# soedinglab/spacedust

Hardware: AMD Instinct MI355X
Metric: clustersearch throughput (genome-pairs/s; SW GCUPS alongside) (higher is better)
Workload: dtype int16

## Files before the change

spacedust_amd/csrc/hip/sd_sw.hip:

```cpp
#include "sd_common.h"
#include <unistd.h>


#include <algorithm>
#include <cmath>
#include <cstring>
#include <memory>
#include <omp.h>
#include <numeric>

#include "../host/sd_host.h"
#include "sd_sw_pk.h"

namespace {

using sdpk::SwTask;

template <int RT>
__global__ void __launch_bounds__(64)
sw_score_kernel(const SwTask *__restrict__ tasks, uint32_t nTasks, const uint8_t *__restrict__ qRes,
                const int8_t *__restrict__ qBias, const uint8_t *__restrict__ tRes, const int8_t *__restrict__ mat,
                int go, int ge, int32_t *__restrict__ out, uint2 *__restrict__ boundary,
                const uint32_t *__restrict__ order ,
                const int8_t *__restrict__ qProf ) {
// ... 601 lines not shown
    int i = qLen - 1, j = tLen - 1, state = 2;
    char *o = bt + tk.btOff + (qLen + tLen + 2);
    int len = 0, ids = 0;
    bool bad = false;
    bool going = have && reached && (i > 0 || j > 0);
    const int sh = grp * 32;
    while (__ballot(going)) {
        {
            const int ii = i - l, jj = j - l;
            bool ok = going && state == 2 && (ii > 0 || jj > 0) && ii >= 0 && jj >= 0;
            int x = ii - band;
            x = x > 0 ? x : 0;
            x = jj - x;
            ok = ok && x >= 0 && x < width_d;
            bool same = false;
            if (ok) {
                const int byte = dirs[(size_t) 16 * ii + (x >> 1)];
                const int code = (x & 1) ? (byte >> 4) : (byte & 15);
                ok = (code & 12) == 0;
                same = sq[ii] == st[jj];
            }
            const uint32_t okMask = (uint32_t) (__ballot(ok) >> sh);
            const uint32_t sameMask = (uint32_t) (__ballot(same) >> sh);
            const int run = okMask == 0xFFFFFFFFu ? 32 : __builtin_ctz(~okMask);
            const uint32_t runMask = run == 32 ? 0xFFFFFFFFu : ((1u << run) - 1u);
            if (l < run) o[-1 - l] = 'M';
            ids += __builtin_popcount(sameMask & runMask);
            i -= run;
            j -= run;
            o -= run;
            len += run;
        }
        if (going && (i > 0 || j > 0)) {
            if (i < 0 || j < 0) bad = true;
            int x = i - band;
            x = x > 0 ? x : 0;
            x = j - x;
            if (x < 0 || x >= width_d) bad = true;
            if (!bad) {
                const int byte = dirs[(size_t) 16 * i + (x >> 1)];
                const int code = (x & 1) ? (byte >> 4) : (byte & 15);
                int dcode;
                const int dE = (code & 1) ? 3 : 2, dF = (code & 2) ? 5 : 4;
                if (state == 0) dcode = dE;
                else if (state == 1) dcode = dF;
                else dcode = (code & 4) ? dE : ((code & 8) ? dF : 1);
                char c;
                switch (dcode) {
                    case 1: ids += (sq[i] == st[j]); --i; --j; state = 2; c = 'M'; break;
                    case 2: --i; state = 0; c = 'I'; break;
                    case 3: --i; state = 2; c = 'I'; break;
                    case 4: --j; state = 1; c = 'D'; break;
                    default: --j; state = 2; c = 'D'; break;
                }
                --o;
                if (l == 0) *o = c;
                len++;
            }
        }
        going = going && !bad && (i > 0 || j > 0);
    }
    if (!have || !reached || l != 0) return;
    if (bad || i != 0 || j != 0) {
        res[2 * id] = -1;
        return;
    }
    ids += (sq[0] == st[0]);
    *--o = 'M';
    len++;
    res[2 * id] = len;
    res[2 * id + 1] = ids;
}

template <int RT, int LW, bool MULTI, bool WIDE, bool SHARED>
void launchScorePk(sd_ctx *ctx, const SwTask *dTasks, const uint32_t *dOrder, uint32_t n, const sd_seqset *q,
                   const sd_seqset *t, const int8_t *dMat, int go, int ge, int32_t *dOut, uint2 *dBound) {
    if (n == 0) return;
    constexpr uint32_t perWave = 2 * (64 / LW);
    dim3 grid((n + perWave - 1) / perWave), block(64);
    hipLaunchKernelGGL((sdpk::sw_score_pk_kernel<RT, LW, MULTI, WIDE, SHARED>), grid, block, 0, ctx->stream, dTasks, n, q->dRes, q->dBias,
                       t->dRes, dMat, go, ge, dOut, dBound, dOrder, (const int8_t *) q->dProf);
}

template <int RT, bool SHARED>
void launchScorePkAligned(sd_ctx *ctx, const SwTask *dTasks, const uint32_t *dOrder, uint32_t n, const sd_seqset *q, const sd_seqset *t,
                          const int8_t *dMat, int go, int ge, int32_t *dOut) {
    if (n == 0) return;
    constexpr uint32_t perWave = 4;
    dim3 grid((n + perWave - 1) / perWave), block(64);
    hipLaunchKernelGGL((sdpk::sw_score_pk_aligned_kernel<RT, SHARED>), grid, block, 0, ctx->stream, dTasks, n, q->dRes, q->dBias, t->dRes,
                       dMat, go, ge, dOut, dOrder, (const int8_t *) q->dProf);
}

int rtClass(int n) {
    if (n <= 128) return 4;
    if (n <= 256) return 8;
    if (n <= 512) return 16;
    return 32;
}

template <int RT>
void launchScore(sd_ctx *ctx, const SwTask *dTasks, uint32_t n, const sd_seqset *q, const sd_seqset *t,
                 const int8_t *dMat, int go, int ge, int32_t *dOut, uint2 *dBound) {
    if (n == 0) return;
    dim3 grid((n + 1) / 2), block(64);
    hipLaunchKernelGGL(sw_score_kernel<RT>, grid, block, 0, ctx->stream, dTasks, n, q->dRes, q->dBias, t->dRes, dMat,
                       go, ge, dOut, dBound, (const uint32_t *) nullptr, (const int8_t *) q->dProf);
}

template <int RT>
void launchScoreIdx(sd_ctx *ctx, const SwTask *dTasks, const uint32_t *dOrder, uint32_t n, const sd_seqset *q,
                    const sd_seqset *t, const int8_t *dMat, int go, int ge, int32_t *dOut, uint2 *dBound) {
    if (n == 0) return;
    dim3 grid((n + 1) / 2), block(64);
    hipLaunchKernelGGL(sw_score_kernel<RT>, grid, block, 0, ctx->stream, dTasks, n, q->dRes, q->dBias, t->dRes, dMat,
                       go, ge, dOut, dBound, dOrder, (const int8_t *) q->dProf);
}

int runScoreTasks(sd_ctx *ctx, std::vector<SwTask> &tasks, const sd_seqset *q, const sd_seqset *t, const int8_t *dMat,
                  int go, int ge, std::vector<int32_t> &hOut, uint32_t nSlots, uint64_t *cells, const char *tag = "a") {
    hOut.assign((size_t) nSlots * 3, 0);
    if (tasks.empty()) return SD_OK;
    HostScope hsAll(ctx, "score.total");
    const size_t n = tasks.size();
    constexpr int NB = 4 * 1024;
    auto keyOf = [](const SwTask &t) {
        const int c = rtClass(t.n);
        const int ci = c == 4 ? 0 : (c == 8 ? 1 : (c == 16 ? 2 : 3));
        return (uint32_t) ci * 1024u + (uint32_t) (1023 - std::min(t.tL >> 4, 1023));
    };
    SwTask *sorted = nullptr;
    SD_HIP(ctx, pinGet(ctx, (std::string("sw.tasks.") + tag).c_str(), n, &sorted));
    uint64_t boundTotal = 0, cellSum = 0;
    size_t classBegin[5] = {0, 0, 0, 0, 0};
    {
        int T = 1;
#pragma omp parallel
        {
#pragma omp single
            T = omp_get_num_threads();
        }
        T = std::max(1, std::min(T, 64));
        std::vector<uint32_t> hist((size_t) T * NB, 0);
#pragma omp parallel num_threads(T) reduction(+ : cellSum)
        {
            const int th = omp_get_thread_num();
            const size_t lo = n * th / T, hi = n * (th + 1) / T;
            uint32_t *hh = &hist[(size_t) th * NB];
            for (size_t i = lo; i < hi; i++) {
                hh[keyOf(tasks[i])]++;
                cellSum += (uint64_t) tasks[i].n * (uint64_t) tasks[i].tL;
            }
        }
        uint64_t run = 0;
        for (int bkt = 0; bkt < NB; bkt++) {
            if ((bkt & 1023) == 0) classBegin[bkt >> 10] = run;
            for (int th = 0; th < T; th++) {
                const uint32_t c = hist[(size_t) th * NB + bkt];
                hist[(size_t) th * NB + bkt] = (uint32_t) run;
                run += c;
            }
        }
        classBegin[4] = run;
#pragma omp parallel num_threads(T)
        {
            const int th = omp_get_thread_num();
            const size_t lo = n * th / T, hi = n * (th + 1) / T;
            uint32_t *hh = &hist[(size_t) th * NB];
            for (size_t i = lo; i < hi; i++) sorted[hh[keyOf(tasks[i])]++] = tasks[i];
        }
    }
    *cells += cellSum;
    for (size_t i = classBegin[3]; i < classBegin[4]; i++) {
        if (sorted[i].n > 1024) {
            sorted[i].boundOff = boundTotal;
            boundTotal += (uint64_t) sorted[i].tL;
        }
    }
    SwTask *dTasks = nullptr;
    int32_t *dOut = nullptr;
    uint2 *dBound = nullptr;
    int32_t *hPin = nullptr;
    SD_HIP(ctx, wsGet(ctx, "sw.tasks", n, &dTasks));
    SD_HIP(ctx, wsGet(ctx, "sw.out", (size_t) nSlots * 3, &dOut));
    SD_HIP(ctx, wsGet(ctx, "sw.bound", std::max<uint64_t>(boundTotal, 1), &dBound));
    SD_HIP(ctx, pinGet(ctx, "sw.hout", (size_t) nSlots * 3, &hPin));
    SD_HIP(ctx, hipMemcpyAsync(dTasks, sorted, n * sizeof(SwTask), hipMemcpyHostToDevice, ctx->stream));
    SD_HIP(ctx, hipMemsetAsync(dOut, 0, (size_t) nSlots * 3 * sizeof(int32_t), ctx->stream));
    static const int classes[4] = {4, 8, 16, 32};
    for (int ci = 0; ci < 4; ci++) {
        const size_t begin = classBegin[ci], end = classBegin[ci + 1];
        if (end == begin) continue;
        const uint32_t cnt = (uint32_t) (end - begin);
        {
            ProfScope ps(ctx, "sw_score");
            switch (classes[ci]) {
                case 4: launchScore<4>(ctx, dTasks + begin, cnt, q, t, dMat, go, ge, dOut, dBound); break;
                case 8: launchScore<8>(ctx, dTasks + begin, cnt, q, t, dMat, go, ge, dOut, dBound); break;
                case 16: launchScore<16>(ctx, dTasks + begin, cnt, q, t, dMat, go, ge, dOut, dBound); break;
                default: launchScore<32>(ctx, dTasks + begin, cnt, q, t, dMat, go, ge, dOut, dBound); break;
            }
        }
        SD_HIP(ctx, hipGetLastError());
    }
    SD_HIP(ctx, hipMemcpyAsync(hPin, dOut, (size_t) nSlots * 3 * sizeof(int32_t), hipMemcpyDeviceToHost, ctx->stream));
    SD_HIP(ctx, sdStreamSync(ctx));
    memcpy(hOut.data(), hPin, (size_t) nSlots * 3 * sizeof(int32_t));
    return SD_OK;
}


constexpr uint32_t N_NARROW_CLASSES = 24;
constexpr uint32_t FIRST_NARROW_MULTI = 21;
constexpr uint32_t N_PK_CLASSES = 14;
constexpr uint32_t FIRST_MULTI_PK = 11;
constexpr uint32_t FIRST_WIDE_CLASS = N_NARROW_CLASSES;
constexpr uint32_t FIRST_INT32_CLASS = FIRST_WIDE_CLASS + N_PK_CLASSES;
constexpr uint32_t N_SCORE_CLASSES = FIRST_INT32_CLASS + 4;
static_assert(N_SCORE_CLASSES < 63, "class boundaries are found by one 64-lane wavefront; six class bits in the pair key");
enum ScoreKernel { SCORE_PK = 0, SCORE_PK_WIDE = 1, SCORE_INT32 = 2 };
constexpr uint32_t KEY_INVALID = N_SCORE_CLASSES * 1024u;
__host__ __device__ __forceinline__ bool scoreClassIsMulti(uint32_t ci) {
    return (ci >= FIRST_NARROW_MULTI && ci < FIRST_WIDE_CLASS) || (ci >= FIRST_WIDE_CLASS + FIRST_MULTI_PK && ci < FIRST_INT32_CLASS);
}
__device__ __forceinline__ uint32_t scoreKey(int n, int tL, int kernel, int wideRowLimit = 800) {
    int ci;
    if (kernel == SCORE_PK_WIDE && min(n, tL) > wideRowLimit) kernel = SCORE_INT32;
    if (kernel == SCORE_INT32 || tL > 65535) {
        ci = FIRST_INT32_CLASS + (n <= 128 ? 0 : (n <= 256 ? 1 : (n <= 512 ? 2 : 3)));
    } else if (kernel == SCORE_PK_WIDE) {
        if (n <= 192) ci = n <= 128 ? 0 : 1;
        else if (n <= 384) ci = 2 + (n - 193) / 32;
        else if (n <= 768) ci = n <= 512 ? 8 : (n <= 640 ? 9 : 10);
        else ci = min((int) FIRST_MULTI_PK + (n + 511) / 512 - 2, 13);
        ci += FIRST_WIDE_CLASS;
    } else {
        if (n <= 128) ci = 0;
        else if (n <= 768) ci = (n + 31) / 32 - 4;
        else ci = min((int) FIRST_NARROW_MULTI + (n + 511) / 512 - 2, (int) FIRST_WIDE_CLASS - 1);
    }
    return (uint32_t) ci * 1024u + (uint32_t) (1023 - min(tL >> 4, 1023));
}

struct DevGateParams {
    int go, ge, matMin, swMode, covMode, wideRowLimit;
    float covThr;
    double evalThr;
    double lambda, K, aI, bI, alphaI, betaI, aJ, bJ, alphaJ, betaJ, sigma, tau, viThr, vjThr, cThr, dbResidues;
};

__device__ double devEvalue(const DevGateParams &e, double y_, double qLen) {
    const double m_ = e.dbResidues, n_ = qLen;
    const double const_val = 0.3989422804014327;
    double tmp = e.aI * y_ + e.bI;
    double m_li_y = m_ - tmp;
    double vi_y = fmax(e.viThr, e.alphaI * y_ + e.betaI);
    double sqrt_vi_y = sqrt(vi_y);
    double m_F = sqrt_vi_y == 0.0 ? 1e100 : m_li_y / sqrt_vi_y;
    double P_m_F = 0.5 * erfc(-sqrt(0.5) * m_F);
    double E_m_F = -const_val * exp(-0.5 * m_F * m_F);
    double p1 = m_li_y * P_m_F - sqrt_vi_y * E_m_F;
    tmp = e.aJ * y_ + e.bJ;
    double n_lj_y = n_ - tmp;
    double vj_y = fmax(e.vjThr, e.alphaJ * y_ + e.betaJ);
    double sqrt_vj_y = sqrt(vj_y);
    double n_F = sqrt_vj_y == 0.0 ? 1e100 : n_lj_y / sqrt_vj_y;
    double P_n_F = 0.5 * erfc(-sqrt(0.5) * n_F);
    double E_n_F = -const_val * exp(-0.5 * n_F * n_F);
    double p2 = n_lj_y * P_n_F - sqrt_vj_y * E_n_F;
    double c_y = fmax(e.cThr, e.sigma * y_ + e.tau);
    double area = p1 * p2 + c_y * (P_m_F * P_n_F);
    return e.K * exp(-e.lambda * y_) * area;
}

__device__ __forceinline__ float devCov(unsigned int startPos, unsigned int endPos, unsigned int len) {
    return (min(len, max(startPos, endPos)) - min(startPos, endPos) + 1) / (float) len;
}
__device__ __forceinline__ bool devHasCoverage(float covThr, int covMode, float qCov, float tCov) {
    switch (covMode) {
        case 0: return (qCov >= covThr) && (tCov >= covThr);
        case 2: return qCov >= covThr;
        case 1: return tCov >= covThr;
        default: return true;
    }
}

__global__ void __launch_bounds__(256)
k_pre_word(uint32_t nPairs, const uint32_t *__restrict__ pairQ, const uint32_t *__restrict__ pairT, const uint16_t *__restrict__ pairDiag,
           const uint32_t *__restrict__ fwdKeys, const uint64_t *__restrict__ qOff, const uint64_t *__restrict__ tOff,
           const uint8_t *__restrict__ qRes, const int8_t *__restrict__ qBias, const uint8_t *__restrict__ tRes, const int8_t *__restrict__ mat,
           const int8_t *__restrict__ qProf, const int32_t *__restrict__ minBias, int matMin, uint8_t *__restrict__ preWord,
           uint32_t *__restrict__ pass1Keys) {
    __shared__ int8_t smat[441];
    for (int x = threadIdx.x; x < 441; x += blockDim.x) smat[x] = mat[x];
    __syncthreads();
    const uint32_t i = blockIdx.x * blockDim.x + threadIdx.x;
    if (i >= nPairs) return;
    uint8_t pw = 0;
    const uint32_t key = fwdKeys[i];
    if (key != KEY_INVALID) {
        const uint64_t qo = qOff[pairQ[i]], to = tOff[pairT[i]];
        const int qL = (int) (qOff[pairQ[i] + 1] - qo), tL = (int) (tOff[pairT[i] + 1] - to);
        if (qL < 32768 && tL < 32768 && pairDiag[i] != 0x8000) {
            const int d = (int) (int16_t) pairDiag[i];
            int q0 = d >= 0 ? d : 0, t0 = d >= 0 ? 0 : -d;
            const int n = min(qL - q0, tL - t0);
            const int need = 255 - (abs(matMin) + abs(minBias[pairQ[i]]));
            int run = 0, best = 0;
            for (int x = 0; x < n && best < need; x++) {
                const int qr = qRes[qo + q0 + x], tr = tRes[to + t0 + x];
                run += qProf ? (int) qProf[(qo + q0 + x) * 21 + tr] : (int) smat[tr * 21 + qr] + (int) qBias[qo + q0 + x];
                run = run < 0 ? 0 : run;
                best = run > best ? run : best;
            }
            pw = best >= need ? 1 : 0;
        }
    }
    preWord[i] = pw;
    pass1Keys[i] = pw ? KEY_INVALID : key;
}

__global__ void __launch_bounds__(256)
// ... 446 lines not shown
    leader[p] = v;
}
__global__ void __launch_bounds__(256)
k_pair_emit(uint32_t n, const uint32_t *__restrict__ keyS, const uint32_t *__restrict__ vals, const uint32_t *__restrict__ runStartOf,
            const uint64_t *__restrict__ pairIdx, uint32_t *__restrict__ order2) {
    const uint32_t p = blockIdx.x * blockDim.x + threadIdx.x;
    if (p >= n || (keyS[p] >> 26) >= FIRST_INT32_CLASS || ((p - runStartOf[p]) & 1u)) return;
    const uint64_t w = pairIdx[p];
    order2[2 * w] = vals[p];
    const bool mate = p + 1 < n && (keyS[p + 1] >> 9) == (keyS[p] >> 9);
    order2[2 * w + 1] = mate ? vals[p + 1] : PAIR_NONE;
}
__global__ void k_pair_bounds(const uint32_t *__restrict__ keyS, uint32_t n, const uint64_t *__restrict__ pairIdx,
                              uint32_t *__restrict__ b, int nb) {
    const int c = threadIdx.x;
    if (c >= nb) return;
    const uint32_t want = (uint32_t) c << 26;
    uint32_t lo = 0, hi = n;
    while (lo < hi) {
        const uint32_t mid = (lo + hi) >> 1;
        if (keyS[mid] < want) lo = mid + 1;
        else hi = mid;
    }
    b[c] = (uint32_t) pairIdx[lo];
}

int devRunScore(sd_ctx *ctx, uint32_t nPairs, const uint32_t *dKeys, const uint32_t *dVals, uint32_t *dKeysSorted,
                uint32_t *dOrder, uint32_t *dBounds, SwTask *dTasks, uint64_t *dScanA, uint64_t *dScanB,
                const sd_seqset *q, const sd_seqset *t, const int8_t *dMat, int go, int ge, int32_t *dOut,
                uint32_t *nValid, const uint32_t *dPairQ ) {
    const unsigned grid = (nPairs + 255) / 256;
    int rc = SD_OK;
    uint32_t *dOrder2 = nullptr, *dPairBounds = nullptr;
    if (dPairQ) {
        uint32_t *dKey2 = nullptr, *dVals2 = nullptr, *dHead = nullptr, *dRunStart = nullptr;
        uint64_t *dPairIdx = nullptr;
        uint8_t *dLeader = nullptr;
        SD_HIP(ctx, wsGet(ctx, "sp.key2", (size_t) nPairs, &dKey2));
        SD_HIP(ctx, wsGet(ctx, "sp.vals2", (size_t) nPairs, &dVals2));
        SD_HIP(ctx, wsGet(ctx, "sp.head", (size_t) nPairs, &dHead));
        SD_HIP(ctx, wsGet(ctx, "sp.runstart", (size_t) nPairs, &dRunStart));
        SD_HIP(ctx, wsGet(ctx, "sp.leader", (size_t) nPairs + 1, &dLeader));
        SD_HIP(ctx, wsGet(ctx, "sp.pairidx", (size_t) nPairs + 1, &dPairIdx));
        const size_t order2Cap = (size_t) 4 * nPairs + 8;
        SD_HIP(ctx, wsGet(ctx, "sp.order2", order2Cap, &dOrder2));
        SD_HIP(ctx, hipMemsetAsync(dOrder2, 0xFF, order2Cap * sizeof(uint32_t), ctx->stream));
        SD_HIP(ctx, wsGet(ctx, "sp.bounds", 64, &dPairBounds));
        hipLaunchKernelGGL(k_pair_keys, dim3(grid), dim3(256), 0, ctx->stream, nPairs, dKeys, dPairQ, dKey2);
        rc = devSortPairs(ctx, dKey2, dKeysSorted, dVals, dVals2, nPairs, 32);
        if (rc != SD_OK) return rc;
        dOrder = dVals2;
        hipLaunchKernelGGL(k_pair_heads, dim3(grid), dim3(256), 0, ctx->stream, nPairs, dKeysSorted, dHead);
        rc = devInclusiveMax(ctx, dHead, dRunStart, nPairs);
        if (rc != SD_OK) return rc;
        hipLaunchKernelGGL(k_pair_leaders, dim3((nPairs + 256) / 256), dim3(256), 0, ctx->stream, nPairs, dKeysSorted, dRunStart, dLeader);
        rc = devExclusiveScan(ctx, (const uint8_t *) dLeader, dPairIdx, (size_t) nPairs + 1);
        if (rc != SD_OK) return rc;
        hipLaunchKernelGGL(k_pair_emit, dim3(grid), dim3(256), 0, ctx->stream, nPairs, dKeysSorted, dVals2, dRunStart, dPairIdx, dOrder2);
        hipLaunchKernelGGL(k_pair_bounds, dim3(1), dim3(64), 0, ctx->stream, dKeysSorted, nPairs, dPairIdx, dPairBounds,
                           (int) FIRST_INT32_CLASS + 1);
        hipLaunchKernelGGL(k_bounds, dim3(1), dim3(64), 0, ctx->stream, dKeysSorted, nPairs, 1u << 26, dBounds, (int) N_SCORE_CLASSES + 1);
    } else {
        rc = devSortPairs(ctx, dKeys, dKeysSorted, dVals, dOrder, nPairs, 16);
        if (rc != SD_OK) return rc;
        hipLaunchKernelGGL(k_bounds, dim3(1), dim3(64), 0, ctx->stream, dKeysSorted, nPairs, 1024u, dBounds, (int) N_SCORE_CLASSES + 1);
    }
    hipLaunchKernelGGL(k_bound_need, dim3(grid), dim3(256), 0, ctx->stream, nPairs, dTasks, dKeys, dScanA);
    SD_HIP(ctx, hipMemsetAsync(dScanA + nPairs, 0, sizeof(uint64_t), ctx->stream));
    rc = devExclusiveScan(ctx, dScanA, dScanB, (size_t) nPairs + 1);
    if (rc != SD_OK) return rc;
    hipLaunchKernelGGL(k_bound_apply, dim3(grid), dim3(256), 0, ctx->stream, nPairs, dTasks, dScanB);
    uint32_t hb[N_SCORE_CLASSES + 1], hpb[FIRST_INT32_CLASS + 1];
    uint64_t boundTotal = 0;
    if (dPairQ) SD_HIP(ctx, sdD2H(ctx, hpb, dPairBounds, sizeof(hpb)));
    SD_HIP(ctx, sdD2H(ctx, hb, dBounds, sizeof(hb)));
    SD_HIP(ctx, sdD2H(ctx, &boundTotal, dScanB + nPairs, sizeof(uint64_t)));
    SD_HIP(ctx, sdStreamSync(ctx));
    *nValid = hb[N_SCORE_CLASSES];
    uint2 *dBound = nullptr;
    SD_HIP(ctx, wsGet(ctx, "sw.bound", std::max<uint64_t>(boundTotal, 1), &dBound));
    for (uint32_t ci = 0; ci < N_SCORE_CLASSES; ci++) {
        const uint32_t begin = hb[ci], cnt = hb[ci + 1] - hb[ci];
        if (cnt == 0) continue;
        static const char *const pkNames[N_PK_CLASSES] = {"rt4x32", "rt6x32", "rt7x32", "rt8x32", "rt9x32", "rt10x32", "rt11x32", "rt12x32",
                                                          "rt8x64", "rt10x64", "rt12x64", "rt8x64s2", "rt8x64s3", "rt8x64sN"};
        static const char *const i32Names[4] = {"sw_score.rt4", "sw_score.rt8", "sw_score.rt16", "sw_score.rt32"};
        const bool shared = dPairQ != nullptr && ci < FIRST_INT32_CLASS;
        const int alignedRT = (ci >= 1 && ci < FIRST_NARROW_MULTI) ? (int) ci + 4 : 0;
        const bool aligned = alignedRT > 0 && (alignedRT <= 12 || shared);
        int generalIdx = 0;
        if (ci >= FIRST_NARROW_MULTI && ci < FIRST_WIDE_CLASS) generalIdx = (int) FIRST_MULTI_PK + (int) (ci - FIRST_NARROW_MULTI);
        else if (alignedRT) generalIdx = alignedRT <= 6 ? 1 : (alignedRT <= 12 ? alignedRT - 5 : (alignedRT <= 16 ? 8 : (alignedRT <= 20 ? 9 : 10)));
        char name[48];
        if (aligned) snprintf(name, sizeof(name), "sw_score_pk.a_seg%d", alignedRT);
        else if (ci < FIRST_WIDE_CLASS) snprintf(name, sizeof(name), "sw_score_pk.%s", pkNames[generalIdx]);
        else if (ci < FIRST_INT32_CLASS) snprintf(name, sizeof(name), "sw_score_pk.w_%s", pkNames[ci - FIRST_WIDE_CLASS]);
        else snprintf(name, sizeof(name), "%s", i32Names[ci - FIRST_INT32_CLASS]);
        ProfScope ps(ctx, name);
        const uint32_t *ord = dOrder + begin;
        uint32_t nOrd = cnt;
        if (shared) {
            ord = dOrder2 + 2 * (size_t) hpb[ci];
            nOrd = 2 * (hpb[ci + 1] - hpb[ci]);
        }
#define SD_PK(RT, LW, MULTI, WIDE)                                                                                          \
    do {                                                                                                                   \
        if (shared) launchScorePk<RT, LW, MULTI, WIDE, true>(ctx, dTasks, ord, nOrd, q, t, dMat, go, ge, dOut, dBound);     \
        else launchScorePk<RT, LW, MULTI, WIDE, false>(ctx, dTasks, ord, nOrd, q, t, dMat, go, ge, dOut, dBound);           \
    } while (0)
#define SD_PKA(RT)                                                                                       \
    case RT:                                                                                             \
        if (shared) launchScorePkAligned<RT, true>(ctx, dTasks, ord, nOrd, q, t, dMat, go, ge, dOut);    \
        else launchScorePkAligned<RT, false>(ctx, dTasks, ord, nOrd, q, t, dMat, go, ge, dOut);          \
        break;
#define SD_PK_CLASS(WIDE, IDX)                                                \
        switch (IDX) {                                                        \
            case 0: SD_PK(4, 32, false, WIDE); break;                         \
            case 1: SD_PK(6, 32, false, WIDE); break;                         \
            case 2: SD_PK(7, 32, false, WIDE); break;                         \
            case 3: SD_PK(8, 32, false, WIDE); break;                         \
            case 4: SD_PK(9, 32, false, WIDE); break;                         \
            case 5: SD_PK(10, 32, false, WIDE); break;                        \
            case 6: SD_PK(11, 32, false, WIDE); break;                        \
            case 7: SD_PK(12, 32, false, WIDE); break;                        \
            case 8: SD_PK(8, 64, false, WIDE); break;                         \
            case 9: SD_PK(10, 64, false, WIDE); break;                        \
            case 10: SD_PK(12, 64, false, WIDE); break;                       \
            default: SD_PK(8, 64, true, WIDE); break;                         \
        }
        if (aligned) {
            switch (alignedRT) {
                SD_PKA(5) SD_PKA(6) SD_PKA(7) SD_PKA(8) SD_PKA(9) SD_PKA(10) SD_PKA(11) SD_PKA(12) SD_PKA(13) SD_PKA(14)
                SD_PKA(15) SD_PKA(16) SD_PKA(17) SD_PKA(18) SD_PKA(19) SD_PKA(20) SD_PKA(21) SD_PKA(22) SD_PKA(23) SD_PKA(24)
                default: break;
            }
        } else if (ci < FIRST_WIDE_CLASS) {
            SD_PK_CLASS(false, generalIdx)
        } else if (ci < FIRST_INT32_CLASS) {
            SD_PK_CLASS(true, (int) (ci - FIRST_WIDE_CLASS))
        } else {
            switch (ci - FIRST_INT32_CLASS) {
                case 0: launchScoreIdx<4>(ctx, dTasks, ord, cnt, q, t, dMat, go, ge, dOut, dBound); break;
                case 1: launchScoreIdx<8>(ctx, dTasks, ord, cnt, q, t, dMat, go, ge, dOut, dBound); break;
                case 2: launchScoreIdx<16>(ctx, dTasks, ord, cnt, q, t, dMat, go, ge, dOut, dBound); break;
                default: launchScoreIdx<32>(ctx, dTasks, ord, cnt, q, t, dMat, go, ge, dOut, dBound); break;
            }
        }
#undef SD_PKA
#undef SD_PK_CLASS
#undef SD_PK
    }
    SD_HIP(ctx, hipGetLastError());
    return SD_OK;
}

__global__ void __launch_bounds__(256)
k_cells(uint32_t nPairs, const SwTask *__restrict__ tasks, const uint32_t *__restrict__ keys, unsigned long long *__restrict__ acc) {
    const uint32_t i = blockIdx.x * blockDim.x + threadIdx.x;
    unsigned long long c = 0;
    if (i < nPairs && keys[i] != KEY_INVALID) c = (unsigned long long) tasks[i].n * (unsigned long long) tasks[i].tL;
#pragma unroll
    for (int off = 32; off >= 1; off >>= 1) c += __shfl_xor(c, off, 64);
    if ((threadIdx.x & 63) == 0 && c) atomicAdd(acc, c);
}

}

int sdFail(sd_ctx *ctx, int code, const char *fmt, ...) {
    char buf[1024];
    va_list ap;
    va_start(ap, fmt);
    vsnprintf(buf, sizeof(buf), fmt, ap);
    va_end(ap);
    if (ctx) ctx->lastError = buf;
    else fprintf(stderr, "spacedust_gpu: %s\n", buf);
    return code;
}

extern "C" {

int sd_ctx_create(int device, sd_ctx **out) { return sd_ctx_create_prio(device, 0, out); }

int sd_ctx_create_prio(int device, int priority, sd_ctx **out) { return sd_ctx_create_masked(device, priority, 0, out); }

int sd_ctx_create_masked(int device, int priority, int reserveCUs, sd_ctx **out) {
    if (out == nullptr) return SD_EINVAL;
    *out = nullptr;
    int count = 0;
    hipError_t e = hipGetDeviceCount(&count);
    if (e != hipSuccess || count <= 0) {
        fprintf(stderr, "spacedust_gpu: no HIP device visible (%s); this library has no CPU fallback\n",
                e != hipSuccess ? hipGetErrorString(e) : "device count 0");
        return SD_ENODEVICE;
    }
    if (device < 0 || device >= count) return SD_EINVAL;
    if (hipSetDevice(device) != hipSuccess) return SD_ENODEVICE;
    sd_ctx *c = new sd_ctx();
    c->device = device;
    int least = 0, greatest = 0;
    (void) hipDeviceGetStreamPriorityRange(&least, &greatest);
    const int prio = priority < 0 ? greatest : (priority > 0 ? least : (least + greatest) / 2);
    hipError_t se = hipSuccess;
    (void) hipGetDeviceProperties(&c->prop, device);
    const int nCU = c->prop.multiProcessorCount;
    if (reserveCUs > 0 && nCU > 0 && reserveCUs < nCU) {
        std::vector<uint32_t> mask((size_t) (nCU + 31) / 32, 0u);
        for (int b = 0; b < nCU - reserveCUs; b++) mask[(size_t) b / 32] |= 1u << (b % 32);
        se = hipExtStreamCreateWithCUMask(&c->stream, (uint32_t) mask.size(), mask.data());
    } else {
        se = hipStreamCreateWithPriority(&c->stream, hipStreamNonBlocking, prio);
    }
    if (se != hipSuccess) {
        delete c;
        return SD_EHIP;
    }
    const char *syncMode = getenv("SD_SYNC");
    const bool spin = syncMode && strcmp(syncMode, "spin") == 0;
    (void) hipEventCreate(&c->evStart);
    (void) hipEventCreate(&c->evStop);
    if (!spin) (void) hipEventCreateWithFlags(&c->evSync, hipEventDisableTiming);
    (void) hipGetDeviceProperties(&c->prop, device);
    *out = c;
    return SD_OK;
}

void sd_ctx_destroy(sd_ctx *ctx) {
    if (!ctx) return;
    (void) hipSetDevice(ctx->device);
    if (ctx->evStart) (void) hipEventDestroy(ctx->evStart);
    if (ctx->evStop) (void) hipEventDestroy(ctx->evStop);
    if (ctx->evSync) (void) hipEventDestroy(ctx->evSync);
// ... 1105 lines not shown
```

spacedust_amd/csrc/hip/sd_sw_pk.h:

```cpp
#ifndef SD_SW_PK_H
#define SD_SW_PK_H

#include <hip/hip_runtime.h>
#include <cstdint>

namespace sdpk {

struct SwTask {
    uint64_t qOff;
    uint64_t tOff;
    int32_t n;
    int32_t tL;
    int32_t qStep;
    int32_t tStep;
    int32_t segLen;
    uint32_t slot;
    uint64_t boundOff;
};

typedef short s16x2 __attribute__((ext_vector_type(2)));
typedef unsigned short u16x2 __attribute__((ext_vector_type(2)));

__device__ __forceinline__ uint32_t pkMax(uint32_t a, uint32_t b) {
    return __builtin_bit_cast(uint32_t, __builtin_elementwise_max(__builtin_bit_cast(s16x2, a), __builtin_bit_cast(s16x2, b)));
// ... 260 lines not shown
                        cm = pkMax(cm, pkRowCode(g, 31 - r));
                    }
                }
                outG = H[RT - 1];
                outFf = Ff;
                outFl = Fl;
                if (MULTI && !lastStrip && l == LW - 1) {
                    const int c = k0 + i - (LW - 1);
                    if (c >= 0 && c < pairTL) {
                        const unsigned long long lo = (unsigned long long) outG | ((unsigned long long) outFf << 32);
                        __hip_atomic_store((unsigned long long *) &bnd[c], lo, __ATOMIC_RELAXED, __HIP_MEMORY_SCOPE_AGENT);
                        __hip_atomic_store((unsigned long long *) &bnd[c] + 1, (unsigned long long) outFl, __ATOMIC_RELAXED,
                                           __HIP_MEMORY_SCOPE_AGENT);
                    }
                }
                if (WIDE) {
                    const bool upA = cmA > (bestA | 0xFFFFu), upB = cmB > (bestB | 0xFFFFu);
                    bestA = upA ? cmA : bestA;
                    bcolA = upA ? ccol : bcolA;
                    bestB = upB ? cmB : bestB;
                    bcolB = upB ? ccol : bcolB;
                } else {
                    const uint32_t v = pkLshr(cm, 5);
                    const uint32_t nb = pkMax(bestv, v);
                    const uint32_t m = pkAshr(pkSub(bestv, nb), 15);
                    bestcm = bfi(m, cm, bestcm);
                    bestcol = bfi(m, ccol, bestcol);
                    bestv = nb;
                }
                ccol = pkAdd(ccol, 0x00010001u);
            }
            chunk = chunkNext;
            bchunk = bnext;
        }
        {
            const uint32_t vA = WIDE ? bestA >> 16 : bestv & 0xFFFFu, vB = WIDE ? bestB >> 16 : bestv >> 16;
            const uint32_t rcA = WIDE ? bestA & 31u : bestcm & 31u, rcB = WIDE ? bestB & 31u : (bestcm >> 16) & 31u;
            const uint32_t rowA = (uint32_t) (q0 + 31 - (int) rcA), rowB = (uint32_t) (q0 + 31 - (int) rcB);
            const uint32_t colA = WIDE ? bcolA & 0xFFFFu : bestcol & 0xFFFFu, colB = WIDE ? bcolB >> 16 : bestcol >> 16;
            if (vA > 0) {
                const unsigned long long kk = ((unsigned long long) vA << 40) | ((unsigned long long) (0xFFFFFu - colA) << 20) |
                                              (unsigned long long) (0xFFFFFu - rowA);
                keyA = kk > keyA ? kk : keyA;
            }
            if (vB > 0) {
                const unsigned long long kk = ((unsigned long long) vB << 40) | ((unsigned long long) (0xFFFFFu - colB) << 20) |
                                              (unsigned long long) (0xFFFFFu - rowB);
                keyB = kk > keyB ? kk : keyB;
            }
        }
    }
#pragma unroll
    for (int off = LW / 2; off >= 1; off >>= 1) {
        const unsigned long long oa = __shfl_xor(keyA, off, LW), ob = __shfl_xor(keyB, off, LW);
        keyA = oa > keyA ? oa : keyA;
        keyB = ob > keyB ? ob : keyB;
    }
    if (l == 0) {
        if (haveA) {
            const int v = (int) (keyA >> 40);
            out[3 * A.slot + 0] = v;
            out[3 * A.slot + 1] = v == 0 ? -1 : 0xFFFFF - (int) ((keyA >> 20) & 0xFFFFF);
            out[3 * A.slot + 2] = v == 0 ? A.n - 1 : 0xFFFFF - (int) (keyA & 0xFFFFF);
        }
        if (haveB) {
            const int v = (int) (keyB >> 40);
            out[3 * B.slot + 0] = v;
            out[3 * B.slot + 1] = v == 0 ? -1 : 0xFFFFF - (int) ((keyB >> 20) & 0xFFFFF);
            out[3 * B.slot + 2] = v == 0 ? B.n - 1 : 0xFFFFF - (int) (keyB & 0xFFFFF);
        }
    }
}

__device__ __forceinline__ uint32_t pkAshr15(uint32_t a) {
    uint32_t r;
    asm("v_pk_ashrrev_i16 %0, 15, %1 op_sel_hi:[0,1]" : "=v"(r) : "v"(a));
    return r;
}
__device__ __forceinline__ uint32_t bfiAsm(uint32_t mask, uint32_t a, uint32_t b) {
    uint32_t r;
    asm("v_bfi_b32 %0, %1, %2, %3" : "=v"(r) : "v"(mask), "v"(a), "v"(b));
    return r;
}
__device__ __forceinline__ uint32_t addWord0(uint32_t base, uint32_t packed) {
    uint32_t r;
    asm("v_add_u32_sdwa %0, %1, %2 dst_sel:DWORD dst_unused:UNUSED_PAD src0_sel:DWORD src1_sel:WORD_0" : "=v"(r) : "v"(base), "v"(packed));
    return r;
}
__device__ __forceinline__ uint32_t addWord1(uint32_t base, uint32_t packed) {
    uint32_t r;
    asm("v_add_u32_sdwa %0, %1, %2 dst_sel:DWORD dst_unused:UNUSED_PAD src0_sel:DWORD src1_sel:WORD_1" : "=v"(r) : "v"(base), "v"(packed));
    return r;
}

template <int RT, bool SHARED>
__global__ void __launch_bounds__(64)
sw_score_pk_aligned_kernel(const SwTask *__restrict__ tasks, uint32_t nTasks, const uint8_t *__restrict__ qRes,
                           const int8_t *__restrict__ qBias, const uint8_t *__restrict__ tRes, const int8_t *__restrict__ mat,
                           int go, int ge, int32_t *__restrict__ out, const uint32_t *__restrict__ order,
                           const int8_t *__restrict__ qProf) {
    constexpr int LW = 32;
    constexpr int WORDS = (RT + 3) / 4;
    constexpr int RTP = 4 * WORDS;
    constexpr int PSTRIDE = LW * WORDS;
    constexpr int NGRP = 64 / LW;
    constexpr int NT = 2 * NGRP;
    constexpr uint32_t ROWB = PSTRIDE * 4;
    static_assert(22 * ROWB < 65536, "row offsets travel in 16 bits");
    __shared__ uint32_t prof[SHARED ? 1 : NT][22][PSTRIDE];
    __shared__ int8_t smat[441];
    for (int i = threadIdx.x; i < 441; i += 64) smat[i] = mat[i];
    __syncthreads();
    const int lane = threadIdx.x & 63, wave = threadIdx.x >> 6;
    const int grp = lane / LW, l = lane % LW;
    SwTask tk[NT];
#pragma unroll
    for (int x = 0; x < NT; x++) {
        const uint32_t id = (blockIdx.x + (uint32_t) wave) * NT + x;
        const uint32_t tid = id < nTasks ? (order ? order[id] : id) : 0xFFFFFFFFu;
        if (tid != 0xFFFFFFFFu) {
            tk[x] = tasks[tid];
        } else {
            tk[x].n = 0; tk[x].tL = 0; tk[x].qOff = 0; tk[x].tOff = 0; tk[x].qStep = 1; tk[x].tStep = 1; tk[x].segLen = 1;
            tk[x].slot = 0; tk[x].boundOff = 0;
        }
    }
    SwTask A = tk[0], B = tk[1];
#pragma unroll
    for (int g = 1; g < NGRP; g++)
        if (grp == g) {
            A = tk[2 * g];
            B = tk[2 * g + 1];
        }
    const bool haveA = A.n > 0, haveB = B.n > 0;
    if (SHARED && !haveB) {
        B = A;
        B.tL = 0;
    }
    int maxN = 0, maxTL = 0;
#pragma unroll
    for (int x = 0; x < NT; x++) {
        maxN = max(maxN, tk[x].n);
        maxTL = max(maxTL, tk[x].tL);
    }
    const int steps = (maxN > 0 && maxTL > 0) ? maxTL + LW - 1 : 0;
    const uint32_t goP = (uint32_t) go | ((uint32_t) go << 16), geP = (uint32_t) ge | ((uint32_t) ge << 16);
    const int q0 = l * RT;
#pragma unroll
    for (int x = 0; x < (SHARED ? 1 : 2); x++) {
        const SwTask &T = SHARED ? tk[0] : (x ? B : A);
        uint32_t *pw = &prof[SHARED ? 0 : 2 * grp + x][0][0] + l * WORDS;
#pragma unroll
        for (int w = 0; w < WORDS; w++) {
            int res[4], cb[4];
            int64_t pidx[4];
            bool valid[4];
#pragma unroll
            for (int b = 0; b < 4; b++) {
                const int qi = q0 + 4 * w + b;
                valid[b] = (4 * w + b < RT) && qi < T.n;
                res[b] = 20;
                cb[b] = 0;
                pidx[b] = 0;
                if (valid[b]) {
                    const int64_t idx = (int64_t) T.qOff + (int64_t) qi * T.qStep;
                    res[b] = qRes[idx];
                    cb[b] = qBias[idx];
                    pidx[b] = idx * 21;
                }
            }
            const int aFirst = SHARED ? wave * NGRP + grp : 0, aStep = SHARED ? NGRP : 1;
            if (qProf) {
                for (int a = aFirst; a < 21; a += aStep) {
                    uint32_t word = 0;
#pragma unroll
                    for (int b = 0; b < 4; b++) {
                        const int v = valid[b] ? (int) qProf[pidx[b] + a] : -64;
                        word |= (uint32_t) (uint8_t) (int8_t) v << (8 * b);
                    }
                    pw[a * PSTRIDE + w] = word;
                }
            } else {
                for (int a = aFirst; a < 21; a += aStep) {
                    uint32_t word = 0;
#pragma unroll
                    for (int b = 0; b < 4; b++) {
                        const int v = valid[b] ? (int) smat[a * 21 + res[b]] + cb[b] : -64;
                        word |= (uint32_t) (uint8_t) (int8_t) v << (8 * b);
                    }
                    pw[a * PSTRIDE + w] = word;
                }
            }
            pw[PK_NEUTRAL * PSTRIDE + w] = 0xC0C0C0C0u;
        }
    }
    __syncthreads();
    typedef __attribute__((address_space(3))) uint32_t lds_u32;
    const uint32_t baseA = (uint32_t) (size_t) (lds_u32 *) (&prof[SHARED ? 0 : 2 * grp][0][0] + l * WORDS);
    const uint32_t baseB = SHARED ? baseA : (uint32_t) (size_t) (lds_u32 *) (&prof[2 * grp + 1][0][0] + l * WORDS);
    auto ldsWord = [](uint32_t addr, int w) -> uint32_t { return *((const lds_u32 *) (size_t) addr + w); };

    uint32_t H[RTP], E[RTP];
#pragma unroll
    for (int r = 0; r < RTP; r++) {
        H[r] = 0;
        E[r] = 0;
    }
    uint32_t outG = 0, outFf = 0, prevInG = 0;
    uint32_t bestcm = 0, bestcol = 0;
    constexpr uint32_t NEUT = (uint32_t) PK_NEUTRAL * ROWB;
    auto loadChunk = [&](int c0) -> uint32_t {
        const int col = c0 + l;
        uint32_t a = PK_NEUTRAL, b = PK_NEUTRAL;
        if (col < A.tL) a = tRes[(int64_t) A.tOff + (int64_t) col * A.tStep];
        if (col < B.tL) b = tRes[(int64_t) B.tOff + (int64_t) col * B.tStep];
        return (a * ROWB) | ((b * ROWB) << 16);
    };
    uint32_t chunk = loadChunk(0);
    uint32_t chunkNext = loadChunk(LW);
    uint32_t T = NEUT | (NEUT << 16);
    T = writeLane<0>(readLane(chunk, 0), T);
    T = writeLane<32>(readLane(chunk, 32), T);
    uint32_t pa[WORDS], pb[WORDS];
    {
        const uint32_t aA = addWord0(baseA, T), aB = addWord1(baseB, T);
#pragma unroll
        for (int w = 0; w < WORDS; w++) {
            pa[w] = ldsWord(aA, w);
            pb[w] = ldsWord(aB, w);
        }
    }
    auto columnStep = [&](const int k, const uint32_t &Tc, const uint32_t (&pac)[WORDS], const uint32_t (&pbc)[WORDS], uint32_t &Tn,
                          uint32_t (&pan)[WORDS], uint32_t (&pbn)[WORDS]) {
        const int i1 = (k + 1) & (LW - 1);
        if (i1 == 0) {
            chunk = chunkNext;
            chunkNext = loadChunk(k + 1 + LW);
        }
        Tn = dppShr1(Tc);
        Tn = writeLane<0>(readLane(chunk, i1), Tn);
        Tn = writeLane<32>(readLane(chunk, 32 + i1), Tn);
        {
            const uint32_t aA = addWord0(baseA, Tn), aB = addWord1(baseB, Tn);
#pragma unroll
            for (int w = 0; w < WORDS; w++) {
                pan[w] = ldsWord(aA, w);
                pbn[w] = ldsWord(aB, w);
            }
        }
        uint32_t inG = dppShr1(outG), inFf = dppShr1(outFf);
        inG = writeLane<32>(0, inG);
        inFf = writeLane<32>(0, inFf);
        uint32_t h[RTP];
#pragma unroll
        for (int w = 0; w < WORDS; w++) {
            const uint32_t d0 = (w == 0) ? prevInG : H[4 * w - 1];
            addProfile4(pac[w], pbc[w], d0, H[4 * w], H[4 * w + 1], H[4 * w + 2], h[4 * w], h[4 * w + 1], h[4 * w + 2], h[4 * w + 3]);
        }
        prevInG = inG;
        uint32_t Fl = 0, Ff = inFf, cm = 0;
#pragma unroll
        for (int r = 0; r < RT; r++) {
            uint32_t hpre = pkMax(h[r], E[r]);
            if (r != 0) hpre = pkMax(hpre, Fl);
            const uint32_t g = pkMax(hpre, Ff);
            const uint32_t open = pkSubSat(hpre, goP);
            E[r] = pkMax(pkSubSat(E[r], geP), open);
            if (r == 0) Fl = open;
            else if (r + 1 != RT) Fl = pkMax(pkSubSat(Fl, geP), open);
            Ff = pkMax(pkSubSat(Ff, geP), open);
            H[r] = g;
            const uint32_t code = pkRowCode(g, 31 - r);
            cm = r == 0 ? code : pkMax(cm, code);
        }
        outG = H[RT - 1];
        outFf = Ff;
        const uint32_t t = bestcm | 0x001F001Fu;
        const uint32_t m = pkAshr15(pkSub(t, cm));
        const uint32_t kk = (uint32_t) k | ((uint32_t) k << 16);
        bestcm = bfiAsm(m, cm, bestcm);
        bestcol = bfiAsm(m, kk, bestcol);
    };
    uint32_t T2, pa2[WORDS], pb2[WORDS];
#pragma unroll 1
    for (int k = 0; k < steps; k += 2) {
        columnStep(k, T, pa, pb, T2, pa2, pb2);
        columnStep(k + 1, T2, pa2, pb2, T, pa, pb);
    }
    unsigned long long keyA = 0, keyB = 0;
    {
        const uint32_t vA = (bestcm & 0xFFFFu) >> 5, vB = bestcm >> 21;
        const uint32_t rowA = (uint32_t) (q0 + 31 - (int) (bestcm & 31u)), rowB = (uint32_t) (q0 + 31 - (int) ((bestcm >> 16) & 31u));
        const uint32_t colA = (bestcol & 0xFFFFu) - (uint32_t) l, colB = (bestcol >> 16) - (uint32_t) l;
        if (vA > 0) keyA = ((unsigned long long) vA << 40) | ((unsigned long long) (0xFFFFFu - colA) << 20) | (unsigned long long) (0xFFFFFu - rowA);
        if (vB > 0) keyB = ((unsigned long long) vB << 40) | ((unsigned long long) (0xFFFFFu - colB) << 20) | (unsigned long long) (0xFFFFFu - rowB);
    }
#pragma unroll
    for (int off = LW / 2; off >= 1; off >>= 1) {
        const unsigned long long oa = __shfl_xor(keyA, off, LW), ob = __shfl_xor(keyB, off, LW);
        keyA = oa > keyA ? oa : keyA;
        keyB = ob > keyB ? ob : keyB;
    }
    if (l == 0) {
        if (haveA) {
            const int v = (int) (keyA >> 40);
            out[3 * A.slot + 0] = v;
            out[3 * A.slot + 1] = v == 0 ? -1 : 0xFFFFF - (int) ((keyA >> 20) & 0xFFFFF);
            out[3 * A.slot + 2] = v == 0 ? A.n - 1 : 0xFFFFF - (int) (keyA & 0xFFFFF);
        }
        if (haveB) {
            const int v = (int) (keyB >> 40);
            out[3 * B.slot + 0] = v;
            out[3 * B.slot + 1] = v == 0 ? -1 : 0xFFFFF - (int) ((keyB >> 20) & 0xFFFFF);
            out[3 * B.slot + 2] = v == 0 ? B.n - 1 : 0xFFFFF - (int) (keyB & 0xFFFFF);
        }
    }
}

}
#endif
```

Baseline: 2647.

## Route wide-score classes through aligned segmented kernel with per-lane-pair row split

Adds a WORD variant of the aligned packed Smith-Waterman kernel, in which each pair of lanes shares one query segment, so wide (16-bit full-score) classes can use the aligned path instead of the general wide kernel. Wide classes now reuse the narrow class binning, and the best-cell tracking gets full 16-bit scores via max3 codes. The intent is to cut the per-column overhead of the general wide kernel for these tasks. In exchange the code carries more complex F-propagation between lanes and odd-segment masking, which adds correctness risk and register pressure.

New measurement: 2632, median of 2. Within noise of the previous version (-0.5%).

```diff
diff --git a/spacedust_amd/csrc/hip/sd_sw.hip b/spacedust_amd/csrc/hip/sd_sw.hip
--- a/spacedust_amd/csrc/hip/sd_sw.hip
+++ b/spacedust_amd/csrc/hip/sd_sw.hip
@@ -707,14 +707,29 @@
                        t->dRes, dMat, go, ge, dOut, dBound, dOrder, (const int8_t *) q->dProf);
 }
 
-template <int RT, bool SHARED>
+template <int RT, bool SHARED, bool WORD>
 void launchScorePkAligned(sd_ctx *ctx, const SwTask *dTasks, const uint32_t *dOrder, uint32_t n, const sd_seqset *q, const sd_seqset *t,
                           const int8_t *dMat, int go, int ge, int32_t *dOut) {
     if (n == 0) return;
     constexpr uint32_t perWave = 4;
     dim3 grid((n + perWave - 1) / perWave), block(64);
-    hipLaunchKernelGGL((sdpk::sw_score_pk_aligned_kernel<RT, SHARED>), grid, block, 0, ctx->stream, dTasks, n, q->dRes, q->dBias, t->dRes,
+    hipLaunchKernelGGL((sdpk::sw_score_pk_aligned_kernel<RT, SHARED, WORD>), grid, block, 0, ctx->stream, dTasks, n, q->dRes, q->dBias, t->dRes,
                        dMat, go, ge, dOut, dOrder, (const int8_t *) q->dProf);
+}
+
+template <int RT>
+void launchScorePkAlignedClass(bool word, bool shared, sd_ctx *ctx, const SwTask *dTasks, const uint32_t *dOrder, uint32_t n,
+                               const sd_seqset *q, const sd_seqset *t, const int8_t *dMat, int go, int ge, int32_t *dOut) {
+    if constexpr (RT <= 12) {
+        if (word && shared) launchScorePkAligned<RT, true, true>(ctx, dTasks, dOrder, n, q, t, dMat, go, ge, dOut);
+        else if (word) launchScorePkAligned<RT, false, true>(ctx, dTasks, dOrder, n, q, t, dMat, go, ge, dOut);
+        else if (shared) launchScorePkAligned<RT, true, false>(ctx, dTasks, dOrder, n, q, t, dMat, go, ge, dOut);
+        else launchScorePkAligned<RT, false, false>(ctx, dTasks, dOrder, n, q, t, dMat, go, ge, dOut);
+    } else {
+        (void) word;
+        (void) shared;
+        launchScorePkAligned<RT, true, false>(ctx, dTasks, dOrder, n, q, t, dMat, go, ge, dOut);
+    }
 }
 
 int rtClass(int n) {
@@ -837,32 +852,25 @@
 
 constexpr uint32_t N_NARROW_CLASSES = 24;
 constexpr uint32_t FIRST_NARROW_MULTI = 21;
-constexpr uint32_t N_PK_CLASSES = 14;
-constexpr uint32_t FIRST_MULTI_PK = 11;
 constexpr uint32_t FIRST_WIDE_CLASS = N_NARROW_CLASSES;
-constexpr uint32_t FIRST_INT32_CLASS = FIRST_WIDE_CLASS + N_PK_CLASSES;
+constexpr uint32_t FIRST_INT32_CLASS = FIRST_WIDE_CLASS + N_NARROW_CLASSES;
 constexpr uint32_t N_SCORE_CLASSES = FIRST_INT32_CLASS + 4;
 static_assert(N_SCORE_CLASSES < 63, "class boundaries are found by one 64-lane wavefront; six class bits in the pair key");
 enum ScoreKernel { SCORE_PK = 0, SCORE_PK_WIDE = 1, SCORE_INT32 = 2 };
 constexpr uint32_t KEY_INVALID = N_SCORE_CLASSES * 1024u;
 __host__ __device__ __forceinline__ bool scoreClassIsMulti(uint32_t ci) {
-    return (ci >= FIRST_NARROW_MULTI && ci < FIRST_WIDE_CLASS) || (ci >= FIRST_WIDE_CLASS + FIRST_MULTI_PK && ci < FIRST_INT32_CLASS);
+    return (ci >= FIRST_NARROW_MULTI && ci < FIRST_WIDE_CLASS) || (ci >= FIRST_WIDE_CLASS + FIRST_NARROW_MULTI && ci < FIRST_INT32_CLASS);
 }
 __device__ __forceinline__ uint32_t scoreKey(int n, int tL, int kernel, int wideRowLimit = 800) {
     int ci;
     if (kernel == SCORE_PK_WIDE && min(n, tL) > wideRowLimit) kernel = SCORE_INT32;
     if (kernel == SCORE_INT32 || tL > 65535) {
         ci = FIRST_INT32_CLASS + (n <= 128 ? 0 : (n <= 256 ? 1 : (n <= 512 ? 2 : 3)));
-    } else if (kernel == SCORE_PK_WIDE) {
-        if (n <= 192) ci = n <= 128 ? 0 : 1;
-        else if (n <= 384) ci = 2 + (n - 193) / 32;
-        else if (n <= 768) ci = n <= 512 ? 8 : (n <= 640 ? 9 : 10);
-        else ci = min((int) FIRST_MULTI_PK + (n + 511) / 512 - 2, 13);
-        ci += FIRST_WIDE_CLASS;
     } else {
         if (n <= 128) ci = 0;
         else if (n <= 768) ci = (n + 31) / 32 - 4;
         else ci = min((int) FIRST_NARROW_MULTI + (n + 511) / 512 - 2, (int) FIRST_WIDE_CLASS - 1);
+        if (kernel == SCORE_PK_WIDE) ci += FIRST_WIDE_CLASS;
     }
     return (uint32_t) ci * 1024u + (uint32_t) (1023 - min(tL >> 4, 1023));
 }
@@ -1475,20 +1483,20 @@
     for (uint32_t ci = 0; ci < N_SCORE_CLASSES; ci++) {
         const uint32_t begin = hb[ci], cnt = hb[ci + 1] - hb[ci];
         if (cnt == 0) continue;
-        static const char *const pkNames[N_PK_CLASSES] = {"rt4x32", "rt6x32", "rt7x32", "rt8x32", "rt9x32", "rt10x32", "rt11x32", "rt12x32",
-                                                          "rt8x64", "rt10x64", "rt12x64", "rt8x64s2", "rt8x64s3", "rt8x64sN"};
         static const char *const i32Names[4] = {"sw_score.rt4", "sw_score.rt8", "sw_score.rt16", "sw_score.rt32"};
         const bool shared = dPairQ != nullptr && ci < FIRST_INT32_CLASS;
-        const int alignedRT = (ci >= 1 && ci < FIRST_NARROW_MULTI) ? (int) ci + 4 : 0;
-        const bool aligned = alignedRT > 0 && (alignedRT <= 12 || shared);
-        int generalIdx = 0;
-        if (ci >= FIRST_NARROW_MULTI && ci < FIRST_WIDE_CLASS) generalIdx = (int) FIRST_MULTI_PK + (int) (ci - FIRST_NARROW_MULTI);
-        else if (alignedRT) generalIdx = alignedRT <= 6 ? 1 : (alignedRT <= 12 ? alignedRT - 5 : (alignedRT <= 16 ? 8 : (alignedRT <= 20 ? 9 : 10)));
+        const bool word = ci >= FIRST_WIDE_CLASS && ci < FIRST_INT32_CLASS;
+        const uint32_t rowCls = word ? ci - FIRST_WIDE_CLASS : ci;
+        const int alignedRT = (ci < FIRST_INT32_CLASS && rowCls >= 1 && rowCls < FIRST_NARROW_MULTI) ? (int) rowCls + 4 : 0;
+        const bool aligned = alignedRT > 0 && (alignedRT <= 12 || (shared && !word));
+        const char *general = rowCls == 0 ? "rt4x32"
+                              : rowCls >= FIRST_NARROW_MULTI ? "rt8x64s"
+                              : alignedRT <= 16 ? "rt8x64" : (alignedRT <= 20 ? "rt10x64" : "rt12x64");
         char name[48];
-        if (aligned) snprintf(name, sizeof(name), "sw_score_pk.a_seg%d", alignedRT);
-        else if (ci < FIRST_WIDE_CLASS) snprintf(name, sizeof(name), "sw_score_pk.%s", pkNames[generalIdx]);
-        else if (ci < FIRST_INT32_CLASS) snprintf(name, sizeof(name), "sw_score_pk.w_%s", pkNames[ci - FIRST_WIDE_CLASS]);
-        else snprintf(name, sizeof(name), "%s", i32Names[ci - FIRST_INT32_CLASS]);
+        if (ci >= FIRST_INT32_CLASS) snprintf(name, sizeof(name), "%s", i32Names[ci - FIRST_INT32_CLASS]);
+        else if (aligned) snprintf(name, sizeof(name), "sw_score_pk.%s%d", word ? "aw_seg" : "a_seg", alignedRT);
+        else if (rowCls >= FIRST_NARROW_MULTI) snprintf(name, sizeof(name), "sw_score_pk.%s%s%s", word ? "w_" : "", general, rowCls == FIRST_NARROW_MULTI ? "2" : (rowCls == FIRST_NARROW_MULTI + 1 ? "3" : "N"));
+        else snprintf(name, sizeof(name), "sw_score_pk.%s%s", word ? "w_" : "", general);
         ProfScope ps(ctx, name);
         const uint32_t *ord = dOrder + begin;
         uint32_t nOrd = cnt;
@@ -1501,26 +1509,21 @@
         if (shared) launchScorePk<RT, LW, MULTI, WIDE, true>(ctx, dTasks, ord, nOrd, q, t, dMat, go, ge, dOut, dBound);     \
         else launchScorePk<RT, LW, MULTI, WIDE, false>(ctx, dTasks, ord, nOrd, q, t, dMat, go, ge, dOut, dBound);           \
     } while (0)
-#define SD_PKA(RT)                                                                                       \
-    case RT:                                                                                             \
-        if (shared) launchScorePkAligned<RT, true>(ctx, dTasks, ord, nOrd, q, t, dMat, go, ge, dOut);    \
-        else launchScorePkAligned<RT, false>(ctx, dTasks, ord, nOrd, q, t, dMat, go, ge, dOut);          \
+#define SD_PKA(RT)                                                                                            \
+    case RT:                                                                                                  \
+        launchScorePkAlignedClass<RT>(word, shared, ctx, dTasks, ord, nOrd, q, t, dMat, go, ge, dOut);        \
         break;
-#define SD_PK_CLASS(WIDE, IDX)                                                \
-        switch (IDX) {                                                        \
-            case 0: SD_PK(4, 32, false, WIDE); break;                         \
-            case 1: SD_PK(6, 32, false, WIDE); break;                         \
-            case 2: SD_PK(7, 32, false, WIDE); break;                         \
-            case 3: SD_PK(8, 32, false, WIDE); break;                         \
-            case 4: SD_PK(9, 32, false, WIDE); break;                         \
-            case 5: SD_PK(10, 32, false, WIDE); break;                        \
-            case 6: SD_PK(11, 32, false, WIDE); break;                        \
-            case 7: SD_PK(12, 32, false, WIDE); break;                        \
-            case 8: SD_PK(8, 64, false, WIDE); break;                         \
-            case 9: SD_PK(10, 64, false, WIDE); break;                        \
-            case 10: SD_PK(12, 64, false, WIDE); break;                       \
-            default: SD_PK(8, 64, true, WIDE); break;                         \
-        }
+#define SD_PK_BEYOND(RT, WIDE)                                                                                              \
+    do {                                                                                                                   \
+        if (WIDE) SD_PK(RT, 64, false, true);                                                                              \
+        else launchScorePk<RT, 64, false, false, false>(ctx, dTasks, ord, nOrd, q, t, dMat, go, ge, dOut, dBound);         \
+    } while (0)
+#define SD_PK_CLASS(WIDE)                                                      \
+        if (rowCls == 0) SD_PK(4, 32, false, WIDE);                            \
+        else if (rowCls >= FIRST_NARROW_MULTI) SD_PK(8, 64, true, WIDE);       \
+        else if (alignedRT <= 16) SD_PK_BEYOND(8, WIDE);                       \
+        else if (alignedRT <= 20) SD_PK_BEYOND(10, WIDE);                      \
+        else SD_PK_BEYOND(12, WIDE);
         if (aligned) {
             switch (alignedRT) {
                 SD_PKA(5) SD_PKA(6) SD_PKA(7) SD_PKA(8) SD_PKA(9) SD_PKA(10) SD_PKA(11) SD_PKA(12) SD_PKA(13) SD_PKA(14)
@@ -1528,9 +1531,9 @@
                 default: break;
             }
         } else if (ci < FIRST_WIDE_CLASS) {
-            SD_PK_CLASS(false, generalIdx)
+            SD_PK_CLASS(false)
         } else if (ci < FIRST_INT32_CLASS) {
-            SD_PK_CLASS(true, (int) (ci - FIRST_WIDE_CLASS))
+            SD_PK_CLASS(true)
         } else {
             switch (ci - FIRST_INT32_CLASS) {
                 case 0: launchScoreIdx<4>(ctx, dTasks, ord, cnt, q, t, dMat, go, ge, dOut, dBound); break;
@@ -1540,6 +1543,7 @@
             }
         }
 #undef SD_PKA
+#undef SD_PK_BEYOND
 #undef SD_PK_CLASS
 #undef SD_PK
     }
diff --git a/spacedust_amd/csrc/hip/sd_sw_pk.h b/spacedust_amd/csrc/hip/sd_sw_pk.h
--- a/spacedust_amd/csrc/hip/sd_sw_pk.h
+++ b/spacedust_amd/csrc/hip/sd_sw_pk.h
@@ -366,6 +366,11 @@
     asm("v_bfi_b32 %0, %1, %2, %3" : "=v"(r) : "v"(mask), "v"(a), "v"(b));
     return r;
 }
+__device__ __forceinline__ uint32_t max3u(uint32_t a, uint32_t b, uint32_t c) {
+    uint32_t r;
+    asm("v_max3_u32 %0, %1, %2, %3" : "=v"(r) : "v"(a), "v"(b), "v"(c));
+    return r;
+}
 __device__ __forceinline__ uint32_t addWord0(uint32_t base, uint32_t packed) {
     uint32_t r;
     asm("v_add_u32_sdwa %0, %1, %2 dst_sel:DWORD dst_unused:UNUSED_PAD src0_sel:DWORD src1_sel:WORD_0" : "=v"(r) : "v"(base), "v"(packed));
@@ -377,7 +382,7 @@
     return r;
 }
 
-template <int RT, bool SHARED>
+template <int RT, bool SHARED, bool WORD>
 __global__ void __launch_bounds__(64)
 sw_score_pk_aligned_kernel(const SwTask *__restrict__ tasks, uint32_t nTasks, const uint8_t *__restrict__ qRes,
                            const int8_t *__restrict__ qBias, const uint8_t *__restrict__ tRes, const int8_t *__restrict__ mat,
@@ -429,11 +434,14 @@
     }
     const int steps = (maxN > 0 && maxTL > 0) ? maxTL + LW - 1 : 0;
     const uint32_t goP = (uint32_t) go | ((uint32_t) go << 16), geP = (uint32_t) ge | ((uint32_t) ge << 16);
-    const int q0 = l * RT;
+    auto firstRow = [&](const SwTask &T) { return WORD ? (l >> 1) * T.segLen + (l & 1) * RT : l * RT; };
+    auto laneRows = [&](const SwTask &T) { return WORD && (l & 1) ? T.segLen - RT : RT; };
+    const int q0A = firstRow(A), q0B = firstRow(B);
 #pragma unroll
     for (int x = 0; x < (SHARED ? 1 : 2); x++) {
         const SwTask &T = SHARED ? tk[0] : (x ? B : A);
         uint32_t *pw = &prof[SHARED ? 0 : 2 * grp + x][0][0] + l * WORDS;
+        const int q0 = firstRow(T), rows = laneRows(T);
 #pragma unroll
         for (int w = 0; w < WORDS; w++) {
             int res[4], cb[4];
@@ -442,7 +450,7 @@
 #pragma unroll
             for (int b = 0; b < 4; b++) {
                 const int qi = q0 + 4 * w + b;
-                valid[b] = (4 * w + b < RT) && qi < T.n;
+                valid[b] = (4 * w + b < rows) && qi < T.n;
                 res[b] = 20;
                 cb[b] = 0;
                 pidx[b] = 0;
@@ -490,8 +498,11 @@
         H[r] = 0;
         E[r] = 0;
     }
-    uint32_t outG = 0, outFf = 0, prevInG = 0;
+    uint32_t outG = 0, outFf = 0, outFl = 0, prevInG = 0;
     uint32_t bestcm = 0, bestcol = 0;
+    uint32_t bestA = 0, bestB = 0, bcolA = 0, bcolB = 0;
+    const uint32_t flIn = WORD && (l & 1) ? 0xFFFFFFFFu : 0u;
+    const uint32_t slotM = WORD && (l & 1) ? ((A.segLen & 1) ? 0x0000FFFFu : 0u) | ((B.segLen & 1) ? 0xFFFF0000u : 0u) : 0u;
     constexpr uint32_t NEUT = (uint32_t) PK_NEUTRAL * ROWB;
     auto loadChunk = [&](int c0) -> uint32_t {
         const int col = c0 + l;
@@ -542,28 +553,58 @@
             addProfile4(pac[w], pbc[w], d0, H[4 * w], H[4 * w + 1], H[4 * w + 2], h[4 * w], h[4 * w + 1], h[4 * w + 2], h[4 * w + 3]);
         }
         prevInG = inG;
-        uint32_t Fl = 0, Ff = inFf, cm = 0;
+        uint32_t Fl = WORD ? dppShr1(outFl) & flIn : 0u, Ff = inFf, cm = 0, cmA = 0, cmB = 0, cA = 0, cB = 0, FfUp = 0;
 #pragma unroll
         for (int r = 0; r < RT; r++) {
             uint32_t hpre = pkMax(h[r], E[r]);
-            if (r != 0) hpre = pkMax(hpre, Fl);
+            if (WORD || r != 0) hpre = pkMax(hpre, Fl);
             const uint32_t g = pkMax(hpre, Ff);
             const uint32_t open = pkSubSat(hpre, goP);
             E[r] = pkMax(pkSubSat(E[r], geP), open);
-            if (r == 0) Fl = open;
-            else if (r + 1 != RT) Fl = pkMax(pkSubSat(Fl, geP), open);
+            if (!WORD && r == 0) Fl = open;
+            else if (WORD || r + 1 != RT) Fl = pkMax(pkSubSat(Fl, geP), open);
+            if (WORD && r + 1 == RT) FfUp = Ff;
             Ff = pkMax(pkSubSat(Ff, geP), open);
             H[r] = g;
-            const uint32_t code = pkRowCode(g, 31 - r);
-            cm = r == 0 ? code : pkMax(cm, code);
-        }
-        outG = H[RT - 1];
-        outFf = Ff;
-        const uint32_t t = bestcm | 0x001F001Fu;
-        const uint32_t m = pkAshr15(pkSub(t, cm));
-        const uint32_t kk = (uint32_t) k | ((uint32_t) k << 16);
-        bestcm = bfiAsm(m, cm, bestcm);
-        bestcol = bfiAsm(m, kk, bestcol);
+            if (WORD) {
+                const uint32_t gc = r + 1 == RT ? g & ~slotM : g;
+                const uint32_t a = (gc << 16) | (uint32_t) (31 - r), b = (gc & 0xFFFF0000u) | (uint32_t) (31 - r);
+                if (r & 1) {
+                    cmA = max3u(cmA, cA, a);
+                    cmB = max3u(cmB, cB, b);
+                } else if (r + 1 == RT) {
+                    cmA = max(cmA, a);
+                    cmB = max(cmB, b);
+                } else {
+                    cA = a;
+                    cB = b;
+                }
+            } else {
+                const uint32_t code = pkRowCode(g, 31 - r);
+                cm = r == 0 ? code : pkMax(cm, code);
+            }
+        }
+        if (WORD) {
+            outG = bfiAsm(slotM, H[RT - 2], H[RT - 1]);
+            outFf = bfiAsm(slotM, FfUp, Ff);
+            outFl = Fl;
+        } else {
+            outG = H[RT - 1];
+            outFf = Ff;
+        }
+        if (WORD) {
+            const bool upA = cmA > (bestA | 0xFFFFu), upB = cmB > (bestB | 0xFFFFu);
+            bestA = upA ? cmA : bestA;
+            bcolA = upA ? (uint32_t) k : bcolA;
+            bestB = upB ? cmB : bestB;
+            bcolB = upB ? (uint32_t) k : bcolB;
+        } else {
+            const uint32_t t = bestcm | 0x001F001Fu;
+            const uint32_t m = pkAshr15(pkSub(t, cm));
+            const uint32_t kk = (uint32_t) k | ((uint32_t) k << 16);
+            bestcm = bfiAsm(m, cm, bestcm);
+            bestcol = bfiAsm(m, kk, bestcol);
+        }
     };
     uint32_t T2, pa2[WORDS], pb2[WORDS];
 #pragma unroll 1
@@ -573,9 +614,11 @@
     }
     unsigned long long keyA = 0, keyB = 0;
     {
-        const uint32_t vA = (bestcm & 0xFFFFu) >> 5, vB = bestcm >> 21;
-        const uint32_t rowA = (uint32_t) (q0 + 31 - (int) (bestcm & 31u)), rowB = (uint32_t) (q0 + 31 - (int) ((bestcm >> 16) & 31u));
-        const uint32_t colA = (bestcol & 0xFFFFu) - (uint32_t) l, colB = (bestcol >> 16) - (uint32_t) l;
+        const uint32_t vA = WORD ? bestA >> 16 : (bestcm & 0xFFFFu) >> 5, vB = WORD ? bestB >> 16 : bestcm >> 21;
+        const uint32_t rcA = WORD ? bestA & 31u : bestcm & 31u, rcB = WORD ? bestB & 31u : (bestcm >> 16) & 31u;
+        const uint32_t rowA = (uint32_t) (q0A + 31 - (int) rcA), rowB = (uint32_t) (q0B + 31 - (int) rcB);
+        const uint32_t colA = (WORD ? bcolA : bestcol & 0xFFFFu) - (uint32_t) l;
+        const uint32_t colB = (WORD ? bcolB : bestcol >> 16) - (uint32_t) l;
         if (vA > 0) keyA = ((unsigned long long) vA << 40) | ((unsigned long long) (0xFFFFFu - colA) << 20) | (unsigned long long) (0xFFFFFu - rowA);
         if (vB > 0) keyB = ((unsigned long long) vB << 40) | ((unsigned long long) (0xFFFFFu - colB) << 20) | (unsigned long long) (0xFFFFFu - rowB);
     }
```
